# ml4ai/mliis

Measured on AMD Instinct MI355X. Metric: inner-loop images/sec (EfficientLab-6-3, 224x224, 5-shot), higher is better.
Workload: dtype f32 (the long-K decoder convs and their filter gradients with every operand split exactly into three bf16 terms on the matrix cores, 6 term products, f32 accumulate: fp32-equivalent products; everything else the fp32 instruction)

## Files before the change

### mliis_amd/csrc/bn.hip

```cpp
#include "common.hpp"
#include "se_wgrad.hpp"
#include "bn_fold.hpp"

namespace mliis {

constexpr int kColThreads = 256;
constexpr int kChanBlock = 32;
constexpr int kRowLanes = 32;
constexpr int kBatch = 4;
constexpr int kPoolRows = 128;
constexpr int kStatsPartialTarget = 256;

struct ColGeom {
  int gx;
  int rows_per_block;
  int nblk;
};

static inline ColGeom col_geom(long long rows_per_seg, int C, int nseg, int target_blocks = 2048) {
  ColGeom g;
  g.gx = ceil_div(C, kChanBlock);
  long long want = target_blocks / ((long long)g.gx * (nseg > 0 ? nseg : 1));
  if (want < 1) want = 1;
  long long rpb = (rows_per_seg + want - 1) / want;
  const long long unit = kRowLanes * kBatch;
  rpb = (rpb + unit - 1) / unit * unit;
  g.rows_per_block = (int)rpb;
  g.nblk = ceil_div(rows_per_seg, rpb);
  return g;
}

template <class Op>
__global__ __launch_bounds__(kColThreads) void colreduce_partial_k(Op op, int rows_per_seg, int C, int rows_per_block, int nblk,
                                                                    float* __restrict__ part) {
  constexpr int NV = Op::NV;
  __shared__ float4 sm[NV][4][8];
  const int t = threadIdx.x;
  const int q = t & 7, rl = t >> 3;
  const int c = blockIdx.y * kChanBlock + q * 4;
  const int seg = blockIdx.z;
  const bool active = c < C;
  float4 acc[NV];
#pragma unroll
  for (int v = 0; v < NV; ++v) acc[v] = f4zero();
  if (active) {
    const int r0 = blockIdx.x * rows_per_block;
    int r1 = r0 + rows_per_block;
    if (r1 > rows_per_seg) r1 = rows_per_seg;
    const long long base = (long long)seg * rows_per_seg;
    int r = r0 + rl;
    typename Op::Raw first[kBatch];
#pragma unroll
    for (int u = 0; u < kBatch; ++u) {
      const int ru = r + u * kRowLanes;
      op.load(seg, base + (ru < r1 ? ru : r0), c, first[u]);
    }
    const typename Op::Ctx ctx = op.ctx(c);
#pragma unroll
    for (int u = 0; u < kBatch; ++u)
      if (r + u * kRowLanes < r1) {
        float4 vals[NV];
        op.eval(ctx, first[u], vals);
#pragma unroll
        for (int v = 0; v < NV; ++v) acc[v] = f4add(acc[v], vals[v]);
// ... 2 lines not shown
    for (; r + (kBatch - 1) * kRowLanes < r1; r += kBatch * kRowLanes) {
      typename Op::Raw raw[kBatch];
#pragma unroll
      for (int u = 0; u < kBatch; ++u) op.load(seg, base + r + u * kRowLanes, c, raw[u]);
#pragma unroll
      for (int u = 0; u < kBatch; ++u) {
        float4 vals[NV];
        op.eval(ctx, raw[u], vals);
#pragma unroll
        for (int v = 0; v < NV; ++v) acc[v] = f4add(acc[v], vals[v]);
      }
    }
    for (; r < r1; r += kRowLanes) {
      typename Op::Raw raw;
      op.load(seg, base + r, c, raw);
      float4 vals[NV];
      op.eval(ctx, raw, vals);
#pragma unroll
      for (int v = 0; v < NV; ++v) acc[v] = f4add(acc[v], vals[v]);
    }
  }
#pragma unroll
  for (int v = 0; v < NV; ++v) {
#pragma unroll
    for (int off = 8; off < 64; off <<= 1) {
      acc[v].x += __shfl_xor(acc[v].x, off);
      acc[v].y += __shfl_xor(acc[v].y, off);
      acc[v].z += __shfl_xor(acc[v].z, off);
      acc[v].w += __shfl_xor(acc[v].w, off);
    }
    if ((t & 63) < 8) sm[v][t >> 6][q] = acc[v];
  }
  __syncthreads();
  if (t < 8 * NV) {
    const int v = t >> 3, qq = t & 7;
    const int cc = blockIdx.y * kChanBlock + qq * 4;
    if (cc < C) {
      float4 s4 = f4add(f4add(sm[v][0][qq], sm[v][1][qq]), f4add(sm[v][2][qq], sm[v][3][qq]));
      st4(part + (((long long)seg * nblk + blockIdx.x) * NV + v) * C + cc, s4);
    }
  }
}

template <class Op>
static int launch_colreduce(Op op, long long rows_per_seg, int C, int nseg, float* part, size_t part_floats,
                            hipStream_t stream, ColGeom* out_g, const char* name, int target_blocks = 2048) {
  ColGeom g = col_geom(rows_per_seg, C, nseg, target_blocks);
  size_t need = (size_t)nseg * g.nblk * Op::NV * C;
  MLIIS_REQUIRE(need <= part_floats, MLIIS_ERR_WORKSPACE, "%s: workspace too small (%zu floats needed, %zu given)", name,
                need, part_floats);
  dim3 grid(g.nblk, g.gx, nseg);
  hipLaunchKernelGGL((colreduce_partial_k<Op>), grid, dim3(kColThreads), 0, stream, op, (int)rows_per_seg, C, g.rows_per_block, g.nblk,
                     part);
  MLIIS_CHECK_LAUNCH(name);
  *out_g = g;
  return MLIIS_OK;
}

struct StatsOp {
  static constexpr int NV = 2;
  const float* x;
  int ld;
  int pre_swish;
  typedef float4 Raw;
  struct Ctx {};
  __device__ __forceinline__ Ctx ctx(int) const { return Ctx(); }
  __device__ __forceinline__ void load(int, long long row, int c, Raw& r) const { r = ld4(x + row * ld + c); }
// ... 437 lines not shown
  }
  __device__ __forceinline__ void eval(const Ctx& k, const Raw& r, float4* o) const {
    float a[5], b[5], c[5], d[5];
    one(r.x.x, r.g.x, k.m.x, k.rs.x, k.ga.x, k.be.x, a);
    one(r.x.y, r.g.y, k.m.y, k.rs.y, k.ga.y, k.be.y, b);
    one(r.x.z, r.g.z, k.m.z, k.rs.z, k.ga.z, k.be.z, c);
    one(r.x.w, r.g.w, k.m.w, k.rs.w, k.ga.w, k.be.w, d);
#pragma unroll
    for (int v = 0; v < 5; ++v) o[v] = make_float4(a[v], b[v], c[v], d[v]);
  }
};

struct Outer2Op {
  static constexpr int NV = 2;
  const float* x;
  int ldx;
  const float* mask;
  const float* dy;
  struct Raw { float4 x, m; float2 d; };
  struct Ctx {};
  __device__ __forceinline__ Ctx ctx(int) const { return Ctx(); }
  __device__ __forceinline__ void load(int, long long row, int c, Raw& r) const {
    r.x = ld4(x + row * ldx + c);
    r.m = mask != nullptr ? ld4(mask + row * ldx + c) : make_float4(1.f, 1.f, 1.f, 1.f);
    r.d = *reinterpret_cast<const float2*>(dy + row * 2);
  }
  __device__ __forceinline__ void eval(const Ctx&, const Raw& r, float4* o) const {
    const float4 v = f4mul(r.x, r.m);
    o[0] = f4scale(v, lone(r.d.x));
    o[1] = f4scale(v, lone(r.d.y));
  }
};

__global__ __launch_bounds__(256) void sum_finalize_k(const float* __restrict__ part, int nblk, int NV, int C, int nseg, float scale,
                                                      float* __restrict__ out, int accumulate) {
  __shared__ double sm[kFoldY * (kFoldX + 1)];
  const int c = blockIdx.x * kFoldX + threadIdx.x;
  const int v = blockIdx.y, seg = blockIdx.z;
  const bool ok = c < C;
  const double s = fold_partials(part + (long long)seg * nblk * NV * C, nblk, (long long)NV * C, (long long)v * C + c, ok, sm);
  if (!ok || threadIdx.y != 0) return;
  const long long i = ((long long)seg * NV + v) * C + c;
  const float r = (float)(s * (double)scale);
  out[i] = accumulate ? out[i] + r : r;
}

constexpr int kFoldTile = 256;

__global__ __launch_bounds__(256) void fold_batched_k(const float* __restrict__ part_base, float* __restrict__ out_base,
                                                      const long long* __restrict__ desc, int ndesc, long long fold_tiles,
                                                      const long long* __restrict__ se_desc, int n_se) {
  __shared__ double sm[3][64][4];
  const long long tile = blockIdx.x;
  if (tile >= fold_tiles) {
    se_wgrad_tile(se_desc, n_se, tile - fold_tiles);
    return;
  }
  int lo = 0, hi = ndesc - 1;
  while (lo < hi) {
    const int mid = (lo + hi + 1) >> 1;
    if (desc[(long long)mid * 8 + 7] <= tile) lo = mid; else hi = mid - 1;
  }
  const long long* d = desc + (long long)lo * 8;
  const long long total = d[2];
  const int nblk = (int)d[6];
  const int t = threadIdx.x, ql = t & 63, sl = t >> 6;
  const long long i = (tile - d[7]) * kFoldTile + ql * 4;
  const bool vec = ((total | d[0]) & 3) == 0;
  const float* p = part_base + d[0] + i;
  double a0 = 0, a1 = 0, a2 = 0, a3 = 0;
  if (i < total) {
    if (vec) {
      int k = sl;
      for (; k + 60 < nblk; k += 64) {
        float4 v[16];
#pragma unroll
        for (int u = 0; u < 16; ++u) v[u] = ld4(p + (long long)(k + 4 * u) * total);
#pragma unroll
        for (int u = 0; u < 16; ++u) { a0 += v[u].x; a1 += v[u].y; a2 += v[u].z; a3 += v[u].w; }
      }
      for (; k + 12 < nblk; k += 16) {
        float4 v[4];
#pragma unroll
        for (int u = 0; u < 4; ++u) v[u] = ld4(p + (long long)(k + 4 * u) * total);
#pragma unroll
        for (int u = 0; u < 4; ++u) { a0 += v[u].x; a1 += v[u].y; a2 += v[u].z; a3 += v[u].w; }
      }
      for (; k < nblk; k += 4) {
        const float4 v = ld4(p + (long long)k * total);
        a0 += v.x; a1 += v.y; a2 += v.z; a3 += v.w;
      }
    } else {
      for (int k = sl; k < nblk; k += 4) {
        const float* pk = p + (long long)k * total;
        a0 += pk[0];
        if (i + 1 < total) a1 += pk[1];
        if (i + 2 < total) a2 += pk[2];
        if (i + 3 < total) a3 += pk[3];
      }
// ... 458 lines not shown
        a1 += (double)d[u].y + (double)d[u].w;
      }
    }
    if ((rows & 1) && t == 0) {
      a0 += dy[(rows - 1) * 2];
      a1 += dy[(rows - 1) * 2 + 1];
    }
    sb[0][t] = a0;
    sb[1][t] = a1;
    __syncthreads();
    for (int s_ = 128; s_ > 0; s_ >>= 1) {
      if (t < s_) {
        sb[0][t] += sb[0][t + s_];
        sb[1][t] += sb[1][t + s_];
      }
      __syncthreads();
    }
    if (t == 0) {
      db[0] = (float)sb[0][0];
      db[1] = (float)sb[1][0];
    }
    return;
  }
  const int c = blockIdx.x * kFoldX + threadIdx.x;
  const int j = blockIdx.y;
  const bool ok = c < C;
  const double s = fold_partials(part, nblk, 2LL * C, (long long)j * C + c, ok, sm);
  if (ok && threadIdx.y == 0) dw[c * 2 + j] = (float)s;
}
}

extern "C" int mliis_final_conv_bwd_filter(const float* x, int ldx, const float* mask, const float* dy, long long rows, int C,
                                           float* dw, float* db, float* ws, size_t ws_floats, hipStream_t stream) {
  MLIIS_REQUIRE(x && dy && dw && db && ws, MLIIS_ERR_ARG, "final_conv_bwd_filter: null pointer");
  MLIIS_REQUIRE(rows > 0 && C > 0 && (C & 3) == 0 && (ldx & 3) == 0 && ldx >= C, MLIIS_ERR_ARG, "final_conv_bwd_filter: bad shape");
  MLIIS_REQUIRE(aligned16(x) && aligned16(mask) && aligned16(ws) && aligned16(dy), MLIIS_ERR_ALIGN, "final_conv_bwd_filter: alignment");
  Outer2Op op{x, ldx, mask, dy};
  ColGeom g;
  int rc = launch_colreduce(op, rows, C, 1, ws, ws_floats, stream, &g, "final_conv_bwd_filter");
  if (rc) return rc;
  hipLaunchKernelGGL(final_dw_finalize_k, dim3(ceil_div(C, kFoldX), 3), dim3(kFoldX, kFoldY), 0, stream, ws, g.nblk, C, dw, dy, rows, db);
  MLIIS_CHECK_LAUNCH("final_dw_finalize");
  return MLIIS_OK;
}
```

### mliis_amd/csrc/se.hip

```cpp
#include "common.hpp"
#include "se_wgrad.hpp"

namespace mliis {

constexpr int kMaxR = 128;
constexpr int kSeThreads = 1024;

template <int U>
__device__ __forceinline__ float dot_strided(const float* __restrict__ a, int sa, const float* __restrict__ b, long long sb, int n) {
  float acc = 0.f;
  for (int i = 0; i < n; i += U) {
    float x[U], y[U];
#pragma unroll
    for (int u = 0; u < U; ++u) {
      const int k = i + u < n ? i + u : n - 1;
      x[u] = a[(long long)k * sa];
      y[u] = b[(long long)k * sb];
    }
#pragma unroll
    for (int u = 0; u < U; ++u) acc = fmaf(i + u < n ? x[u] : 0.f, y[u], acc);
  }
  return acc;
}

// ... 303 lines not shown
    const long long r = ru;
    const long long n = ru / (unsigned)rows_per_img;
    float* dst = y + r * ldy + c;
    const float4 vx = ld4(x ? x + r * ldx + c : dst);
    const float4 vs = ld4(S ? S + n * C + c : dst);
    const float4 va = ld4(A ? A + n * C + c : dst);
    const float4 vo = ld4(dst);
    float4 v = x ? vx : f4zero();
    if (S) v = f4mul(v, vs);
    if (A) v = f4add(v, va);
    if (accumulate) v = f4add(v, vo);
    st4(dst, v);
  }
}

__global__ __launch_bounds__(256) void chan_split_k(const float* __restrict__ x, int ldx, const float* __restrict__ A, float* __restrict__ y0,
                                                    int ld0, int c0, int acc0, float* __restrict__ y1, int ld1, int acc1, long long rows, int C,
                                                    int rows_per_img) {
  const unsigned Q = (unsigned)C >> 2;
  const unsigned total = (unsigned)rows * Q;
  for (unsigned i = blockIdx.x * blockDim.x + threadIdx.x; i < total; i += gridDim.x * blockDim.x) {
    const unsigned ru = i / Q;
    const int c = (int)(i - ru * Q) << 2;
    const long long r = ru;
    const long long n = ru / (unsigned)rows_per_img;
    const bool first = c < c0;
    float* dst = first ? y0 + r * ld0 + c : y1 + r * ld1 + (c - c0);
    const bool acc = first ? acc0 != 0 : acc1 != 0;
    const float4 vx = ld4(x + r * ldx + c);
    const float4 va = ld4(A ? A + n * C + c : x + r * ldx + c);
    const float4 vo = ld4(dst);
    float4 v = vx;
    if (A) v = f4add(v, va);
    if (acc) v = f4add(v, vo);
    st4(dst, v);
  }
}

}

using namespace mliis;

extern "C" {

int mliis_se_mlp_fwd(const float* s_part, int chunks, float scale, float* s_out, const float* w1, const float* b1, const float* w2,
                     const float* b2, float* hpre, float* gate, int N, int C, int R, hipStream_t stream) {
  MLIIS_REQUIRE(s_part && w1 && b1 && w2 && b2 && hpre && gate, MLIIS_ERR_ARG, "se_mlp_fwd: null pointer");
  MLIIS_REQUIRE(N > 0 && C > 0 && C <= 8192 && R > 0 && R <= kMaxR && chunks > 0, MLIIS_ERR_ARG, "se_mlp_fwd: bad shape (R <= %d, C <= 8192)",
                kMaxR);
  const int CL = kSeThreads / R;
  if (C <= kSeThreads && R <= 32 && (C + CL - 1) / CL <= kSeFastDot)
    hipLaunchKernelGGL(se_mlp_fwd_k<true>, dim3(N), dim3(kSeThreads), (size_t)C * sizeof(float), stream, s_part, chunks, scale, s_out, w1, b1, w2,
                       b2, hpre, gate, C, R);
  else
    hipLaunchKernelGGL(se_mlp_fwd_k<false>, dim3(N), dim3(kSeThreads), (size_t)C * sizeof(float), stream, s_part, chunks, scale, s_out, w1, b1, w2,
                       b2, hpre, gate, C, R);
  MLIIS_CHECK_LAUNCH("se_mlp_fwd");
  return MLIIS_OK;
}

int mliis_se_mlp_bwd(const float* dgate, int dgate_row_groups, const float* gate, const float* s, const float* hpre, const float* w1,
                     const float* w1t, const float* w2, float* dpre1, float* dpre2, float* chan_add, float* dw1, float* db1, float* dw2, float* db2, int N,
                     int C, int R, int HW, hipStream_t stream) {
  MLIIS_REQUIRE(dgate_row_groups == 0 || (HW >= 16 && (long long)dgate_row_groups * 16 >= (long long)N * HW), MLIIS_ERR_ARG,
                "se_mlp_bwd: the row-group partials do not cover the N * HW rows (maps of at least 16 pixels)");
  MLIIS_REQUIRE(dgate && gate && s && hpre && w1 && w2 && dpre1 && dpre2 && chan_add, MLIIS_ERR_ARG, "se_mlp_bwd: null pointer (w1t alone may be NULL)");
// ... 16 lines not shown
}

int mliis_se_mlp_bwd_bn(const float* sums, int sums_nblk, const float* gate, const float* hpre, const float* w1, const float* w1t, const float* w2,
                        float* dpre1, float* dpre2, float* chan_add, float* stage1, int N, int C, int R, int HW, hipStream_t stream) {
  MLIIS_REQUIRE(sums && sums_nblk > 0 && gate && hpre && w1 && w2 && dpre1 && dpre2 && chan_add && stage1, MLIIS_ERR_ARG, "se_mlp_bwd_bn: null pointer");
  MLIIS_REQUIRE(N > 0 && C > 0 && C <= 8192 && R > 0 && R <= kMaxR && HW > 0, MLIIS_ERR_ARG, "se_mlp_bwd_bn: bad shape (R <= %d, C <= 8192)", kMaxR);
  if (C <= kSeThreads && R <= 32)
    hipLaunchKernelGGL(se_mlp_bwd_k<true>, dim3(N), dim3(kSeThreads), (size_t)(5 * C + 5 * kSeThreads) * sizeof(float), stream, nullptr, 0, HW, gate, hpre, w1,
                       w1t, w2, dpre2,
                       dpre1, chan_add, C, R, 1.0f / (float)HW, sums, sums_nblk, stage1);
  else
    hipLaunchKernelGGL(se_mlp_bwd_k<false>, dim3(N), dim3(kSeThreads), (size_t)5 * C * sizeof(float), stream, nullptr, 0, HW, gate, hpre, w1, w1t, w2, dpre2,
                       dpre1, chan_add, C, R, 1.0f / (float)HW, sums, sums_nblk, stage1);
  MLIIS_CHECK_LAUNCH("se_mlp_bwd_bn");
  return MLIIS_OK;
}

int mliis_se_wgrad_batched(const long long* desc, int ndesc, long long total_tiles, hipStream_t stream) {
  MLIIS_REQUIRE(desc && ndesc > 0 && total_tiles > 0, MLIIS_ERR_ARG, "se_wgrad_batched: bad arguments");
  hipLaunchKernelGGL(se_wgrad_batched_k, dim3((unsigned)total_tiles), dim3(256), 0, stream, desc, ndesc);
  MLIIS_CHECK_LAUNCH("se_wgrad_batched");
  return MLIIS_OK;
}

int mliis_chan_split(const float* x, int ldx, const float* A, float* y0, int ld0, int c0, int accumulate0, float* y1, int ld1, int accumulate1,
                     long long rows, int C, int rows_per_img, hipStream_t stream) {
  MLIIS_REQUIRE(x && y0 && y1, MLIIS_ERR_ARG, "chan_split: null pointer");
  MLIIS_REQUIRE(rows > 0 && C > 0 && (C & 3) == 0 && c0 > 0 && c0 < C && (c0 & 3) == 0 && (ldx & 3) == 0 && ldx >= C && (ld0 & 3) == 0 &&
                    ld0 >= c0 && (ld1 & 3) == 0 && ld1 >= C - c0 && rows_per_img > 0,
                MLIIS_ERR_ARG, "chan_split: bad shape");
  MLIIS_REQUIRE(aligned16(x) && aligned16(A) && aligned16(y0) && aligned16(y1), MLIIS_ERR_ALIGN, "chan_split: pointers must be 16-byte aligned");
  MLIIS_REQUIRE(rows * (C / 4) < (1LL << 31), MLIIS_ERR_UNSUPPORTED, "chan_split: tensor too large for 32-bit indexing");
  long long q = rows * (C / 4);
  int blocks = (int)((q + 255) / 256 > 4096 ? 4096 : (q + 255) / 256);
  hipLaunchKernelGGL(chan_split_k, dim3(blocks), dim3(256), 0, stream, x, ldx, A, y0, ld0, c0, accumulate0, y1, ld1, accumulate1, rows, C,
                     rows_per_img);
  MLIIS_CHECK_LAUNCH("chan_split");
  return MLIIS_OK;
}

int mliis_chan_affine(const float* x, int ldx, const float* S, const float* A, float* y, int ldy, long long rows, int C,
                      int rows_per_img, int accumulate, hipStream_t stream) {
  MLIIS_REQUIRE(y && (x || A), MLIIS_ERR_ARG, "chan_affine: need an output and at least one of x / A");
  MLIIS_REQUIRE(rows > 0 && C > 0 && (C & 3) == 0 && (ldy & 3) == 0 && ldy >= C && rows_per_img > 0 &&
                    (x == nullptr || ((ldx & 3) == 0 && ldx >= C)),
                MLIIS_ERR_ARG, "chan_affine: bad shape");
  MLIIS_REQUIRE(aligned16(x) && aligned16(S) && aligned16(A) && aligned16(y), MLIIS_ERR_ALIGN, "chan_affine: pointers must be 16-byte aligned");
  MLIIS_REQUIRE(rows * (C / 4) < (1LL << 31), MLIIS_ERR_UNSUPPORTED, "chan_affine: tensor too large for 32-bit indexing");
  long long q = rows * (C / 4);
  int blocks = (int)((q + 255) / 256 > 4096 ? 4096 : (q + 255) / 256);
  hipLaunchKernelGGL(chan_affine_k, dim3(blocks), dim3(256), 0, stream, x, ldx, S, A, y, ldy, rows, C, rows_per_img, accumulate);
  MLIIS_CHECK_LAUNCH("chan_affine");
  return MLIIS_OK;
}
}
```

### mliis_amd/ops.py

```python
from __future__ import annotations

import ctypes as C
import os
from typing import Optional, Tuple

import torch

from ._lib import MliisError, lib
from .spec import BN_EPS, BN_MOMENTUM, MEAN_RGB, STDDEV_RGB

_MEAN3 = (C.c_float * 3)(*MEAN_RGB)
_STD3 = (C.c_float * 3)(*STDDEV_RGB)


def _stream() -> int:
    return torch.cuda.current_stream().cuda_stream


def _ptr(t: Optional[torch.Tensor]):
    if t is None:
        return None
    if not t.is_cuda:
        raise MliisError("mliis_amd ops need device tensors (no CPU path)")
    if t.dtype == torch.bfloat16:
# ... 1001 lines not shown
    lib.call("mliis_resize_bilinear_bwd", _ptr(dy), lddy, _ptr(out), lddx, N, Hi, Wi, Ho, Wo, C_, int(accumulate), _stream())
    return out


def final_conv_fwd(x, w, b, mask=None, out=None):
    rows, C_, ldx = rows_ld(x)
    _dense(w, b, mask)
    if mask is not None and mask.numel() != rows * C_:
        raise MliisError("final_conv_fwd: mask must be a dense [rows, {}] tensor, got {}".format(C_, tuple(mask.shape)))
    _out_dense(out, tuple(x.shape[:-1]) + (2,), what="final_conv_fwd out")
    out = torch.empty(tuple(x.shape[:-1]) + (2,), dtype=torch.float32, device=x.device) if out is None else out
    lib.call("mliis_final_conv_fwd", _ptr(x), ldx, _ptr(mask), _ptr(w), _ptr(b), _ptr(out), rows, C_, _stream())
    return out


def final_conv_bwd_data(dy, w, C_, mask=None, out=None, fin=None):
    rows = dy.numel() // 2
    _dense(dy, w, mask)
    if mask is not None and mask.numel() != rows * C_:
        raise MliisError("final_conv_bwd_data: mask must be a dense [rows, {}] tensor, got {}".format(C_, tuple(mask.shape)))
    _out_rows(out, tuple(dy.shape[:-1]) + (C_,), what="final_conv_bwd_data out")
    out = torch.empty(tuple(dy.shape[:-1]) + (C_,), dtype=torch.float32, device=dy.device) if out is None else out
    _, _, lddx = rows_ld(out)
    if fin is not None:
        buf, size, extra_loss, loss_out = fin
        N, Hd, Wd = dy.shape[:3]
        lib.call("mliis_final_conv_bwd_data_fin", _ptr(dy), _ptr(w), _ptr(mask), _ptr(out), lddx, rows, C_, _ptr(buf), N, Hd, Wd, int(size[0]), int(size[1]),
                 float(extra_loss), _ptr(loss_out), _stream())
        return out
    lib.call("mliis_final_conv_bwd_data", _ptr(dy), _ptr(w), _ptr(mask), _ptr(out), lddx, rows, C_, _stream())
    return out


def final_conv_bwd_filter(x, dy, mask=None, dw=None, db=None, ws: Optional[Workspace] = None):
    rows, C_, ldx = rows_ld(x)
    _dense(dy, mask)
    if mask is not None and mask.numel() != rows * C_:
        raise MliisError("final_conv_bwd_filter: mask must be a dense [rows, {}] tensor, got {}".format(C_, tuple(mask.shape)))
    _out_dense(dw, (1, 1, C_, 2), what="final_conv_bwd_filter dw")
    _out_dense(db, (2,), what="final_conv_bwd_filter db")
    dw = torch.empty((1, 1, C_, 2), dtype=torch.float32, device=x.device) if dw is None else dw
    db = torch.empty(2, dtype=torch.float32, device=x.device) if db is None else db
    ws = ws or default_ws()
    buf = ws.get(lib.size("mliis_colreduce_workspace_floats", rows, C_, 1, 2))
    lib.call("mliis_final_conv_bwd_filter", _ptr(x), ldx, _ptr(mask), _ptr(dy), rows, C_, _ptr(dw), _ptr(db), _ptr(buf), buf.numel(), _stream())
    return dw, db


def softmax_ce(logits, labels, idx=None, label_smoothing=0.0, dice=False, extra_loss=0.0, want_grad=True, want_pred=False, dlogits=None,
               pred=None, out=None, ws: Optional[Workspace] = None):
    N, H, W, _ = logits.shape
    dev = logits.device
    _dense(logits, labels, idx)
    _out_dense(dlogits, tuple(logits.shape), what="softmax_ce dlogits")
    _out_dense(pred, tuple(logits.shape), what="softmax_ce pred")
    if want_grad and dlogits is None:
        dlogits = torch.empty_like(logits)
    if want_pred and pred is None:
        pred = torch.empty_like(logits)
    out = torch.empty(4, dtype=torch.float32, device=dev) if out is None else out
    ws = ws or default_ws()
    buf = ws.get(lib.size("mliis_softmax_ce_workspace_floats", N, H, W))
    lib.call("mliis_softmax_ce", _ptr(logits), _ptr(labels), _ptr(idx), N, H, W, float(label_smoothing), int(dice), float(extra_loss),
             _ptr(dlogits) if want_grad else None, _ptr(pred) if want_pred else None, _ptr(out), _ptr(buf), buf.numel(), _stream())
    return out, dlogits, pred


def head_ce_fused(small, labels, idx, size, label_smoothing, dsmall, out, extra_loss=0.0, ws: Optional[Workspace] = None, finalize=True):
    N, Hd, Wd, _ = small.shape
    _dense(small, labels, idx)
    _out_dense(dsmall, tuple(small.shape), what="head_ce_fused dsmall")
# ... 82 lines not shown
```

### mliis_amd/passes.py

```python
from __future__ import annotations

import torch

from . import ops, spec
from ._lib import MliisError
from .plan import _Plan


class _Pass:

    def __init__(self, L, P: _Plan, training: bool):
        self.L, self.P, self.training = L, P, training
        self.w, self.mv, self.g, self.ws = L.arena.w, L.arena.mv, L.arena.g, L.ws

    def moving(self, prefix):
        return self.mv[prefix + "/moving_mean"], self.mv[prefix + "/moving_variance"]

    def bn_bwd_args(self, st, prefix):
        return st[0], st[1], self.w[prefix + "/gamma"], self.w[prefix + "/beta"]

    def bn_fwd_args(self, st, prefix, moving=True):
        return (self.w[prefix + "/gamma"], self.w[prefix + "/beta"], st[0], st[1]) + (self.moving(prefix) if moving else (None, None))

    def moving_stats(self, st, prefix):
# ... 264 lines not shown
        a, A, ws, T, N = self.arch, self.arena, self.ws, P.aspp, P.N
        w, g = A.w, A.g
        d, hw = a.aspp_dimension, a.aspp_h * a.aspp_h
        (k0, c0), (k1, c1), (k2, c2), (ko, co) = self.n_aspp
        m = T["masks"]
        cat, dcat = T["cat"], T["dcat"]
        dzo = ops.swish_mask_bwd(T["dout"], T["zo"], m[3], out=T["dzo"])
        self._conv_bwd_filter(cat, dzo, 1, 1, out=g[ko], ws=ws)
        ops.colsum(dzo, out=g[co], ws=ws)
        self._conv_bwd_data(dzo, w[ko], 1, out=dcat, ws=ws)
        d0 = ops.swish_mask_bwd(dcat[..., 2 * d:], T["z0"], m[0], out=dcat[..., 2 * d:])
        self._conv_bwd_filter(x, d0, 1, 1, out=g[k0], ws=ws)
        ops.colsum(d0, out=g[c0], ws=ws)
        self._conv_bwd_data(d0, w[k0], 1, out=dx, accumulate=dx_has, ws=ws)
        d1 = ops.swish_mask_bwd(dcat[..., d:2 * d], T["z1"], m[1], out=dcat[..., d:2 * d])
        self._conv_bwd_filter(x, d1, 3, spec.ASPP_DILATION, out=g[k1], ws=ws)
        ops.colsum(d1, out=g[c1], ws=ws)
        self._conv_bwd_data(d1, w[k1], spec.ASPP_DILATION, out=dx, accumulate=True, ws=ws)
        ops.colsum(dcat[..., :d], None, nseg=N, out=T["db2"], ws=ws)
        d2 = ops.swish_mask_bwd(T["db2"], T["z2"], m[2], out=T["db2"], pre_mask=True)
        pool4, d24 = T["pool"].view(N, 1, 1, -1), d2.view(N, 1, 1, d)
        self._conv_bwd_filter(pool4, d24, 1, 1, out=g[k2], ws=ws)
        ops.colsum(d2, out=g[c2], ws=ws)
        self._conv_bwd_data(d24, w[k2], 1, out=T["dpool"].view(N, 1, 1, -1), ws=ws)
        ops.axpby(0.0, None, 1.0 / hw, T["dpool"])
        ops.chan_affine(None, A=T["dpool"], out=dx, accumulate=True)

    def _backward(self, P: _Plan, x, idx, head_fused: bool = False):
        a, S = self.arch, _Pass(self, P, True)
        w, g = S.w, S.g
        if not head_fused:
            ops.resize_bilinear_bwd(P.dlogits, (a.h_dec, a.h_dec), out=P.dsmall)
        mask = P.drop_mask
        ops.final_conv_bwd_filter(P.dec_in, P.dsmall, mask, dw=g[self.n_final[0]], db=g[self.n_final[1]], ws=S.ws)
        has_grad = [False] * len(P.blocks)
        dtop, _ = self._deep_grad_target(P, has_grad, len(a.rsd))
        ops.final_conv_bwd_data(P.dsmall, w[self.n_final[0]], a.c_final, mask, out=dtop, fin=P.head_fin if head_fused else None)
        if not P.wbatch_ready:
            P.wbatch = ops.FilterBatch(self.device)
        for j in range(len(a.rsd) - 1, -1, -1):
            self._rsd_bwd(S, j, has_grad)
        if a.skipdec is not None:
            self._skipdec_bwd(S, has_grad)
        if a.aspp:
            bi = a.reductions[4]
            self._aspp_backward(P, P.blocks[bi]["out"], P.blocks[bi]["dout"], has_grad[bi])
            has_grad[bi] = True
        stage1 = None
        ex = a.executed()
        for bi in range(len(P.blocks) - 1, -1, -1):
            b, B, nm = ex[bi], P.blocks[bi], self.n_blocks[bi]
            if not has_grad[bi]:
                raise MliisError("internal: block {} has no upstream gradient".format(bi))
            tgt = P.blocks[bi - 1]["dout"] if bi > 0 else P.dstem
            tgt_has = has_grad[bi - 1] if bi > 0 else False
            if B["small"]:
                stage1 = self._mbconv_small_bwd(S, bi, b, B, nm, tgt, tgt_has, stage1)
            elif B["march"]:
                stage1 = self._mbconv_march_bwd(S, bi, b, B, nm, tgt, tgt_has, stage1)
            else:
                stage1 = self._mbconv_opbyop_bwd(S, bi, b, B, nm, tgt, tgt_has, stage1)
            if bi > 0:
                has_grad[bi - 1] = True
        self._stem_bwd(S, x, idx, stage1)
        P.wbatch_ready = True
        P.wbatch.launch("fp32x3" if self.x3 is not None else self.matmul_precision)
        ops.fold_batched(P.fold_buf, self.arena.grad, P.fold_desc, P.fold_tiles, se_desc=P.se_desc, se_tiles=P.se_tiles)

    def _deep_grad_target(self, P: _Plan, has_grad, j):
        a = self.arch
        if j > 0:
            return P.rsd[j - 1]["dout"], False
        if j == 0 and a.skipdec is not None:
            return P.skipdec["dout"], False
        if a.aspp:
            return P.aspp["dout"], False
        bi = a.reductions[4]
        tgt_has, has_grad[bi] = has_grad[bi], True
        return P.blocks[bi]["dout"], tgt_has

    def _rsd_bwd(self, S: _Pass, j, has_grad):
        a, P, w, g, ws = self.arch, S.P, S.w, S.g, S.ws
        m, D, nm = a.rsd[j], P.rsd[j], self.n_rsd[j]
        (k0, b0, n0), (k1, b1, n1), (kf, bf, nf) = nm
        co = m.c_out
        dO, cat, pyr, dpyr, dcat = D["dout"], D["cat"], D["pyr"], D["dpyr"], D["dcat"]
        S.bn_b(D["zf"], dO, D["stf"], nf, D["dzf"], pre=True)
        ops.rsd_pool_bwd(D["dzf"], D["tot"], D["pool"], w[kf], 2 * co, dw=g[kf], dbias=g[bf], dpool=D["dpool"], ws=ws)
        S.wgrad_conv(pyr, D["dzf"], 3, 1, kf)
        S.conv_bwd_data(D["dzf"], kf, 1, 2 * co, dpyr)
        d0, d1 = dpyr[..., :co], dpyr[..., co:2 * co]
        ops.bn_bwd_pair([(D["z" + i], d_, *S.bn_bwd_args(D["st" + i], nn), d_, g[nn + "/gamma"], g[nn + "/beta"], P.fold_part[bb])
                         for i, d_, nn, bb in (("0", d0, n0, b0), ("1", d1, n1, b1))], pre_swish=True, ws=ws)
        tail = P.filter_tail[j]
        cmain = cat[..., :m.c_cat - tail] if tail else cat

        def wgrad(dz, kname, kk, dil, cmain=cmain, ctail=cat[..., m.c_cat - tail:] if tail else None):
            S.wgrad_conv(cmain, dz, kk, dil, kname)
            if ctail is not None:
                S.wgrad_conv(ctail, dz, kk, dil, kname + "#tail")
        wgrad(d0, k0, 1, 1)
        self._conv_bwd_data(d0, w[k0], 1, out=dcat, ws=ws)
        wgrad(d1, k1, 3, 2)
        S.conv_bwd_data(d1, k1, 2, m.c_cat, dcat, accumulate=True)
        bi_skip = a.reductions[m.scope_index + 1]
        if m.upsample_conv:
            ku, bu, nu = self.n_rsd_up[j]
            S.bn_b(D["zu"], dO, D["stu"], nu, D["dzu"], pre=True, dxsum_part=P.fold_part[bu])
            S.wgrad_conv(cat[..., :m.c_deep], D["dzu"], 1, 1, ku)
            self._conv_bwd_data(D["dzu"], w[ku], 1, out=D["dup"], ws=ws)
            dU = D["dup"]
        else:
            dU = dO
        ops.chan_split(dcat, m.c_deep, dU, True, P.blocks[bi_skip]["dout"], has_grad[bi_skip], A=D["dpool"])
        has_grad[bi_skip] = True
        tgt, tgt_has = self._deep_grad_target(P, has_grad, j)
        if m.h_in == m.h:
            ops.chan_affine(dU, out=tgt, accumulate=tgt_has)
        else:
            ops.resize_bilinear_bwd(dU, (m.h_in, m.h_in), out=tgt, accumulate=tgt_has)

    def _skipdec_bwd(self, S: _Pass, has_grad):
        a, P, w, ws = self.arch, S.P, S.w, S.ws
        sd, T = a.skipdec, P.skipdec
        (k0, n0), seps = self.n_skipdec
        d = T["dout"]
        for Q, (dwn, dbn, pwn, pbn) in zip(reversed(T["sep"]), reversed(seps)):
            S.bn_b(Q["zp"], d, Q["stp"], pbn, d, post=True)
            S.wgrad_conv(Q["ad"], d, 1, 1, pwn)
            self._conv_bwd_data(d, w[pwn], 1, out=Q["dad"], ws=ws)
            S.bn_b(Q["zd"], Q["dad"], Q["std"], dbn, Q["dad"], post=True)
            ops.dwconv_bwd_filter(Q["x_in"], Q["dad"], 3, 1, partial=P.fold_part[dwn])
            ops.dwconv_bwd_data(Q["dad"], w[dwn], 1, (sd.h, sd.h), out=Q["din"])
            d = Q["din"]
        bi2 = a.reductions[2]
        S.bn_b(T["z0"], d[..., sd.c_in:], T["st0"], n0, T["dz0"], post=True)
        S.wgrad_conv(P.blocks[bi2]["out"], T["dz0"], 1, 1, k0)
        self._conv_bwd_data(T["dz0"], w[k0], 1, out=P.blocks[bi2]["dout"], accumulate=has_grad[bi2], ws=ws)
# ... 96 lines not shown
```

### mliis_amd/plan.py

```python
from __future__ import annotations

import torch

from . import ops, spec
from ._lib import MliisError, lib


class _Plan:

    def __init__(self, L: "Learner", N: int, act_dtype=torch.float32):
        a, dev = L.arch, L.device
        self.N = N
        self.act_dtype = act_dtype

        def buf(*shape):
            return torch.empty(shape, dtype=torch.float32, device=dev)

        def xbuf(*shape):
            return torch.empty(shape, dtype=act_dtype, device=dev)

        def vec(c):
            return buf(c), buf(c)
        self.idx = torch.zeros(N, dtype=torch.int32, device=dev)
        H = a.image_size
# ... 89 lines not shown
        if a.skipdec is not None:
            rows = N * a.skipdec.h ** 2
            for c in (a.skipdec.c_skip, a.skipdec.c_cat, a.skipdec.c_sep):
                need = max(need, -(-rows // 16) * 2 * c, ops.bn_stats_partial_floats(rows, c))
        need = max(need, ops.bn_stats_partial_floats(N * hs * hs, a.stem_out), ops.stem_conv_fwd_stats_floats(N, H, H, a.stem_out))
        self.stats_part = buf(need + 64)
        need2 = 0
        for b in a.executed():
            need2 = max(need2, lib.raw("mliis_dwconv_bn_fwd_blocks")(N, b.h_in, b.h_in, b.cexp, b.k, b.stride) * 2 * b.cexp,
                        lib.raw("mliis_dwconv_bn_bwd_blocks")(N, b.h_in, b.h_in, b.cexp, b.k, b.stride) * 2 * b.cexp)
        for m in a.rsd:
            need2 = max(need2, -(-(N * m.h * m.h) // 16) * 2 * m.c_out, ops.bn_stats_partial_floats(N * m.h * m.h, m.c_out))
        self.stats_part2 = buf(need2 + 64)
        ex_ = a.executed()
        self.bn2_deferred = [bool(L.fuse_bn2 and i + 1 < len(ex_) and ex_[i + 1].expand != 1 and act_dtype in (torch.float32, torch.bfloat16) and
                                  ops.conv2d_fwd_bnin_ok(N, ex_[i].h_out, ex_[i].h_out, ex_[i].cout, ex_[i + 1].cexp)) for i in range(len(ex_))]
        self.stats_part3 = buf(max([-(-(N * b.h_out ** 2) // 16) * 2 * b.cout for b, d in zip(ex_, self.bn2_deferred) if d] + [0]) + 64)
        self.sums_part = buf(max([ops.se_bn_bwd_sums_floats(N, b.h_out * b.h_out, b.cexp) for b in a.executed()] + [0]) + 64)
        self.stage1_se = buf(max([2 * N * b.cexp for b in a.executed()] + [0]) + 64)
        self.pool_part = buf(max(N * (-(-(b.h_out * b.h_out) // 128)) * b.cexp for b in a.executed()) + 64)
        self.gate_part = buf(max([(-(-(N * b.h_out * b.h_out) // 16)) * 2 * b.cexp for b in a.executed() if 16 <= b.h_out * b.h_out <= 256]
                                 + [0]) + 64)
        A = L.arena
        regs, rows, off, tile = {}, [], 0, 0
        fold_tile = lib.raw("mliis_fold_tile_outputs")()

        def add(name, ws_floats, total, seg=None, key=None):
            nonlocal off, tile
            seg_len, seg_stride, seg_off = seg or (total, 0, 0)
            regs[key or name] = (off, ws_floats)
            rows.append([off, A.t_off[name], total, seg_len, seg_stride, seg_off, ws_floats // total, tile])
            off += (ws_floats + 3) // 4 * 4
            tile += -(-total // fold_tile)
        fe = a.name
        add(f"{fe}/stem/conv2d/kernel", lib.size("mliis_stem_conv_bwd_filter_workspace_floats", N, H, H, a.stem_out), 27 * a.stem_out)
        for b, nm, B in zip(a.executed(), L.n_blocks, self.blocks):
            ce = b.cexp
            if b.expand != 1:
                add(nm["w_exp"], lib.size("mliis_conv2d_bwd_filter_workspace_floats", N, b.h_in, b.h_in, b.cin, ce, 1), b.cin * ce)
            if B["march"]:
                add(nm["w_dw"], lib.raw("mliis_dwconv_bn_bwd_blocks")(N, b.h_in, b.h_in, ce, b.k, b.stride) * b.k * b.k * ce, b.k * b.k * ce)
            elif not B["small"]:
                add(nm["w_dw"], lib.size("mliis_dwconv_bwd_filter_workspace_floats", N, b.h_in, b.h_in, ce, b.k, b.stride), b.k * b.k * ce)
            add(nm["w_proj"], lib.size("mliis_conv2d_bwd_filter_workspace_floats", N, b.h_out, b.h_out, ce, b.cout, 1), ce * b.cout)
        if a.skipdec is not None:
            sd, h = a.skipdec, a.skipdec.h
            ksk, seps = L.n_skipdec
            add(ksk[0], lib.size("mliis_conv2d_bwd_filter_workspace_floats", N, h, h, sd.c_skip_in, sd.c_skip, 1), sd.c_skip_in * sd.c_skip)
            cin = sd.c_cat
            for (dwn, _, pwn, _) in seps:
                add(dwn, lib.size("mliis_dwconv_bwd_filter_workspace_floats", N, h, h, cin, 3, 1), 9 * cin)
                add(pwn, lib.size("mliis_conv2d_bwd_filter_workspace_floats", N, h, h, cin, sd.c_sep, 1), cin * sd.c_sep)
                cin = sd.c_sep
        self.filter_tail = {}
        for j_rsd, (m, nm) in enumerate(zip(a.rsd, L.n_rsd)):
            (k0, b0_, _), (k1, b1_, _), (kf, _, _) = nm
            co = m.c_out
            if m.upsample_conv:
                ku, bu, _ = L.n_rsd_up[j_rsd]
                add(ku, lib.size("mliis_conv2d_bwd_filter_workspace_floats", N, m.h, m.h, m.c_deep, co, 1), m.c_deep * co)
                add(bu, ops.bn_bwd_dxsum_floats(N * m.h * m.h, co), co)
            for bias in (b0_, b1_):
                add(bias, ops.bn_bwd_dxsum_floats(N * m.h * m.h, co), co)
            tail = m.c_cat % 64 if (m.c_cat > 64 and 0 < m.c_cat % 64 <= 16) else 0
            self.filter_tail[j_rsd] = tail
            for kk, kname in ((1, k0), (3, k1)):
                main_c = m.c_cat - tail
                add(kname, lib.size("mliis_conv2d_bwd_filter_workspace_floats", N, m.h, m.h, main_c, co, kk), kk * kk * main_c * co,
                    seg=(main_c * co, m.c_cat * co, 0) if tail else None)
                if tail:
                    add(kname, lib.size("mliis_conv2d_bwd_filter_workspace_floats", N, m.h, m.h, tail, co, kk), kk * kk * tail * co,
                        seg=(tail * co, m.c_cat * co, main_c * co), key=kname + "#tail")
            add(kf, lib.size("mliis_conv2d_bwd_filter_workspace_floats", N, m.h, m.h, 2 * co, co, 3), 9 * 2 * co * co,
                seg=(2 * co * co, m.c_pyr * co, 0))
        rows_se, se_tile = [], 0
        for b, B, nm in zip(a.executed(), self.blocks, L.n_blocks):
            se = nm["se"]
            rows_se.append([B["s"].data_ptr(), B["hpre"].data_ptr(), B["dpre1"].data_ptr(), B["dpre2"].data_ptr()] +
                           [A.g[k].data_ptr() for k in se] + [N, b.cexp, b.se, se_tile])
            se_tile += -(-(2 * b.cexp * b.se + b.cexp + b.se) // 256)
        self.se_desc = torch.tensor(rows_se, dtype=torch.int64, device=dev)
        self.se_tiles = se_tile
        self.fold_buf = buf(off + 16)
        self.fold_part = {k: self.fold_buf[o:o + n] for k, (o, n) in regs.items()}
        self.fold_desc = torch.tensor(rows, dtype=torch.int64, device=dev)
        self.fold_tiles = tile
        self.graphs = {}
        self.steps_run = 0
        self.wbatch = ops.FilterBatch(dev)
        self.wbatch_ready = False
        jobs = []
        if L.drop_connect and nskip:
            jobs.append((self.dc_all, L._dc_keeps, N, True))
        if self.drop_mask is not None:
            jobs.append((self.drop_mask, L.drop_keep_dev, self.drop_mask.numel(), False))
        if self.aspp is not None:
            for mbuf in self.aspp["masks"]:
                jobs.append((mbuf, 1.0 - spec.ASPP_DROPOUT, 1, False))
        self.mask_plan = ops.MaskPlan(jobs) if jobs else None

    @property
    def graph(self):
        for g in self.graphs.values():
            return g
        return None
```

Baseline: 3586.

## Fold final conv filter partials in batched fold and fuse direct RSD skip grads

The final 1x1 conv filter gradient now writes its per-block partial slabs, including the bias sums as an extra vector, straight into the shared fold buffer. A new tiny-total path in fold_batched_k reduces them there, which removes the separate finalize launch. The RSD backward, when there is no upsampling and the resolutions match, now routes the skip gradient through bn_b's dskip output. It also adds a chan_split variant that writes both channel halves into one target, summing them in a single pass. Together these cut kernel launches and intermediate buffer traffic, at the cost of more special-case code paths.

After: 3596, median of 6. About the same (+0.3%).

```diff
diff --git a/mliis_amd/csrc/bn.hip b/mliis_amd/csrc/bn.hip
--- a/mliis_amd/csrc/bn.hip
+++ b/mliis_amd/csrc/bn.hip
@@ -30,6 +30,11 @@
   return g;
 }
 
+template <class Op, class = void>
+struct StoresFinalSlabs { static constexpr bool value = false; };
+template <class Op>
+struct StoresFinalSlabs<Op, decltype((void)Op::kFinalSlabs)> { static constexpr bool value = true; };
+
 template <class Op>
 __global__ __launch_bounds__(kColThreads) void colreduce_partial_k(Op op, int rows_per_seg, int C, int rows_per_block, int nblk,
                                                                     float* __restrict__ part) {
@@ -98,7 +103,23 @@
     if ((t & 63) < 8) sm[v][t >> 6][q] = acc[v];
   }
   __syncthreads();
-  if (t < 8 * NV) {
+  if constexpr (StoresFinalSlabs<Op>::value) {
+    if (t < 8) {
+      const int cc = blockIdx.y * kChanBlock + t * 4;
+      if (cc < C) {
+        const float4 s0 = f4add(f4add(sm[0][0][t], sm[0][1][t]), f4add(sm[0][2][t], sm[0][3][t]));
+        const float4 s1 = f4add(f4add(sm[1][0][t], sm[1][1][t]), f4add(sm[1][2][t], sm[1][3][t]));
+        float* o = part + ((long long)blockIdx.x * C + cc) * 2;
+        st4(o, make_float4(s0.x, s1.x, s0.y, s1.y));
+        st4(o + 4, make_float4(s0.z, s1.z, s0.w, s1.w));
+      }
+    } else if (t == 8 && blockIdx.y == 0) {
+      const float4 s2 = f4add(f4add(sm[2][0][0], sm[2][1][0]), f4add(sm[2][2][0], sm[2][3][0]));
+      float* o = part + (long long)nblk * 2 * C + (long long)blockIdx.x * 2;
+      o[0] = s2.x;
+      o[1] = s2.y;
+    }
+  } else if (t < 8 * NV) {
     const int v = t >> 3, qq = t & 7;
     const int cc = blockIdx.y * kChanBlock + qq * 4;
     if (cc < C) {
@@ -602,6 +623,15 @@
   }
 };
 
+struct Outer2SlabOp : Outer2Op {
+  static constexpr int NV = 3;
+  static constexpr bool kFinalSlabs = true;
+  __device__ __forceinline__ void eval(const Ctx& k, const Raw& r, float4* o) const {
+    Outer2Op::eval(k, r, o);
+    o[2] = make_float4(r.d.x, r.d.y, 0.f, 0.f);
+  }
+};
+
 __global__ __launch_bounds__(256) void sum_finalize_k(const float* __restrict__ part, int nblk, int NV, int C, int nseg, float scale,
                                                       float* __restrict__ out, int accumulate) {
   __shared__ double sm[kFoldY * (kFoldX + 1)];
@@ -635,6 +665,27 @@
   const long long total = d[2];
   const int nblk = (int)d[6];
   const int t = threadIdx.x, ql = t & 63, sl = t >> 6;
+  if (total <= 4) {
+    double a[4] = {0.0, 0.0, 0.0, 0.0};
+    for (int k = t; k < nblk; k += 256) {
+      const float* pk = part_base + d[0] + (long long)k * total;
+#pragma unroll
+      for (int e = 0; e < 4; ++e)
+        if (e < total) a[e] += pk[e];
+    }
+#pragma unroll
+    for (int e = 0; e < 4; ++e) {
+#pragma unroll
+      for (int off = 1; off < 64; off <<= 1) a[e] += __shfl_xor(a[e], off);
+      if (ql == 0) sm[0][sl][e] = a[e];
+    }
+    __syncthreads();
+    if (t < total) {
+      const long long seg_len = d[3];
+      out_base[d[1] + (t / seg_len) * d[4] + d[5] + t % seg_len] = (float)((sm[0][0][t] + sm[0][1][t]) + (sm[0][2][t] + sm[0][3][t]));
+    }
+    return;
+  }
   const long long i = (tile - d[7]) * kFoldTile + ql * 4;
   const bool vec = ((total | d[0]) & 3) == 0;
   const float* p = part_base + d[0] + i;
@@ -1159,9 +1210,20 @@
 
 extern "C" int mliis_final_conv_bwd_filter(const float* x, int ldx, const float* mask, const float* dy, long long rows, int C,
                                            float* dw, float* db, float* ws, size_t ws_floats, hipStream_t stream) {
-  MLIIS_REQUIRE(x && dy && dw && db && ws, MLIIS_ERR_ARG, "final_conv_bwd_filter: null pointer");
+  MLIIS_REQUIRE(x && dy && ws && (dw == nullptr) == (db == nullptr), MLIIS_ERR_ARG, "final_conv_bwd_filter: null pointer (dw and db come together)");
   MLIIS_REQUIRE(rows > 0 && C > 0 && (C & 3) == 0 && (ldx & 3) == 0 && ldx >= C, MLIIS_ERR_ARG, "final_conv_bwd_filter: bad shape");
   MLIIS_REQUIRE(aligned16(x) && aligned16(mask) && aligned16(ws) && aligned16(dy), MLIIS_ERR_ALIGN, "final_conv_bwd_filter: alignment");
+  if (dw == nullptr) {
+    const ColGeom gs = col_geom(rows, C, 1);
+    const size_t need = (size_t)gs.nblk * (2 * (size_t)C + 2);
+    MLIIS_REQUIRE(need <= ws_floats, MLIIS_ERR_WORKSPACE, "final_conv_bwd_filter: slab buffer too small (%zu floats needed, %zu given)", need, ws_floats);
+    Outer2SlabOp sop;
+    sop.x = x; sop.ldx = ldx; sop.mask = mask; sop.dy = dy;
+    hipLaunchKernelGGL((colreduce_partial_k<Outer2SlabOp>), dim3(gs.nblk, gs.gx, 1), dim3(kColThreads), 0, stream, sop, (int)rows, C, gs.rows_per_block,
+                       gs.nblk, ws);
+    MLIIS_CHECK_LAUNCH("final_conv_bwd_filter (slabs)");
+    return MLIIS_OK;
+  }
   Outer2Op op{x, ldx, mask, dy};
   ColGeom g;
   int rc = launch_colreduce(op, rows, C, 1, ws, ws_floats, stream, &g, "final_conv_bwd_filter");
diff --git a/mliis_amd/csrc/se.hip b/mliis_amd/csrc/se.hip
--- a/mliis_amd/csrc/se.hip
+++ b/mliis_amd/csrc/se.hip
@@ -359,6 +359,33 @@
     const float4 vo = ld4(dst);
     float4 v = vx;
     if (A) v = f4add(v, va);
+    if (acc) v = f4add(v, vo);
+    st4(dst, v);
+  }
+}
+
+__global__ __launch_bounds__(256) void chan_split_same_k(const float* __restrict__ x, int ldx, const float* __restrict__ A, float* __restrict__ y,
+                                                         int ldy, int c0, int acc, long long rows, int C, int rows_per_img) {
+  const int c1 = C - c0;
+  const unsigned Q = (unsigned)(c0 > c1 ? c0 : c1) >> 2;
+  const unsigned total = (unsigned)rows * Q;
+  for (unsigned i = blockIdx.x * blockDim.x + threadIdx.x; i < total; i += gridDim.x * blockDim.x) {
+    const unsigned ru = i / Q;
+    const int c = (int)(i - ru * Q) << 2;
+    const long long r = ru;
+    const long long n = ru / (unsigned)rows_per_img;
+    const bool h0 = c < c0, h1 = c < c1;
+    const int ca = h0 ? c : c0 + c, cb = h1 ? c0 + c : c;
+    float* dst = y + r * ldy + c;
+    const float4 xa = ld4(x + r * ldx + ca), xb = ld4(x + r * ldx + cb);
+    const float4 aa = ld4(A ? A + n * C + ca : x + r * ldx + ca), ab = ld4(A ? A + n * C + cb : x + r * ldx + cb);
+    const float4 vo = ld4(dst);
+    float4 va = xa, vb = xb;
+    if (A) {
+      va = f4add(va, aa);
+      vb = f4add(vb, ab);
+    }
+    float4 v = h0 ? (h1 ? f4add(va, vb) : va) : vb;
     if (acc) v = f4add(v, vo);
     st4(dst, v);
   }
@@ -441,6 +468,15 @@
   MLIIS_REQUIRE(aligned16(x) && aligned16(A) && aligned16(y0) && aligned16(y1), MLIIS_ERR_ALIGN, "chan_split: pointers must be 16-byte aligned");
   MLIIS_REQUIRE(rows * (C / 4) < (1LL << 31), MLIIS_ERR_UNSUPPORTED, "chan_split: tensor too large for 32-bit indexing");
   long long q = rows * (C / 4);
+  if (y0 == y1) {
+    MLIIS_REQUIRE(ld0 == ld1 && (accumulate0 != 0) == (accumulate1 != 0), MLIIS_ERR_ARG,
+                  "chan_split: y0 == y1 needs one leading dimension and one accumulate setting");
+    q = rows * ((c0 > C - c0 ? c0 : C - c0) / 4);
+    hipLaunchKernelGGL(chan_split_same_k, dim3((int)((q + 255) / 256 > 4096 ? 4096 : (q + 255) / 256)), dim3(256), 0, stream, x, ldx, A, y0, ld0, c0,
+                       accumulate0, rows, C, rows_per_img);
+    MLIIS_CHECK_LAUNCH("chan_split (one target)");
+    return MLIIS_OK;
+  }
   int blocks = (int)((q + 255) / 256 > 4096 ? 4096 : (q + 255) / 256);
   hipLaunchKernelGGL(chan_split_k, dim3(blocks), dim3(256), 0, stream, x, ldx, A, y0, ld0, c0, accumulate0, y1, ld1, accumulate1, rows, C,
                      rows_per_img);
diff --git a/mliis_amd/ops.py b/mliis_amd/ops.py
--- a/mliis_amd/ops.py
+++ b/mliis_amd/ops.py
@@ -1057,11 +1057,21 @@
     return out
 
 
-def final_conv_bwd_filter(x, dy, mask=None, dw=None, db=None, ws: Optional[Workspace] = None):
+def final_conv_bwd_filter_slabs(rows, C_):
+    nb = lib.size("mliis_colreduce_workspace_floats", rows, C_, 1, 2) // (2 * C_)
+    return nb, nb * (2 * C_ + 2)
+
+
+def final_conv_bwd_filter(x, dy, mask=None, dw=None, db=None, ws: Optional[Workspace] = None, slabs=None):
     rows, C_, ldx = rows_ld(x)
-    _dense(dy, mask)
+    _dense(dy, mask, slabs)
     if mask is not None and mask.numel() != rows * C_:
         raise MliisError("final_conv_bwd_filter: mask must be a dense [rows, {}] tensor, got {}".format(C_, tuple(mask.shape)))
+    if slabs is not None:
+        if dw is not None or db is not None:
+            raise MliisError("final_conv_bwd_filter: slabs are folded by fold_batched -- dw / db are not written by this form")
+        lib.call("mliis_final_conv_bwd_filter", _ptr(x), ldx, _ptr(mask), _ptr(dy), rows, C_, None, None, _ptr(slabs), slabs.numel(), _stream())
+        return final_conv_bwd_filter_slabs(rows, C_)[0]
     _out_dense(dw, (1, 1, C_, 2), what="final_conv_bwd_filter dw")
     _out_dense(db, (2,), what="final_conv_bwd_filter db")
     dw = torch.empty((1, 1, C_, 2), dtype=torch.float32, device=x.device) if dw is None else dw
diff --git a/mliis_amd/passes.py b/mliis_amd/passes.py
--- a/mliis_amd/passes.py
+++ b/mliis_amd/passes.py
@@ -320,7 +320,7 @@
         if not head_fused:
             ops.resize_bilinear_bwd(P.dlogits, (a.h_dec, a.h_dec), out=P.dsmall)
         mask = P.drop_mask
-        ops.final_conv_bwd_filter(P.dec_in, P.dsmall, mask, dw=g[self.n_final[0]], db=g[self.n_final[1]], ws=S.ws)
+        ops.final_conv_bwd_filter(P.dec_in, P.dsmall, mask, slabs=P.final_slabs)
         has_grad = [False] * len(P.blocks)
         dtop, _ = self._deep_grad_target(P, has_grad, len(a.rsd))
         ops.final_conv_bwd_data(P.dsmall, w[self.n_final[0]], a.c_final, mask, out=dtop, fin=P.head_fin if head_fused else None)
@@ -373,7 +373,10 @@
         (k0, b0, n0), (k1, b1, n1), (kf, bf, nf) = nm
         co = m.c_out
         dO, cat, pyr, dpyr, dcat = D["dout"], D["cat"], D["pyr"], D["dpyr"], D["dcat"]
-        S.bn_b(D["zf"], dO, D["stf"], nf, D["dzf"], pre=True)
+        direct = m.h_in == m.h and not m.upsample_conv
+        if direct:
+            tgt, tgt_has = self._deep_grad_target(P, has_grad, j)
+        S.bn_b(D["zf"], dO, D["stf"], nf, D["dzf"], pre=True, dskip=tgt if direct else None, dskip_accumulate=direct and tgt_has)
         ops.rsd_pool_bwd(D["dzf"], D["tot"], D["pool"], w[kf], 2 * co, dw=g[kf], dbias=g[bf], dpool=D["dpool"], ws=ws)
         S.wgrad_conv(pyr, D["dzf"], 3, 1, kf)
         S.conv_bwd_data(D["dzf"], kf, 1, 2 * co, dpyr)
@@ -392,6 +395,10 @@
         wgrad(d1, k1, 3, 2)
         S.conv_bwd_data(d1, k1, 2, m.c_cat, dcat, accumulate=True)
         bi_skip = a.reductions[m.scope_index + 1]
+        if direct:
+            ops.chan_split(dcat, m.c_deep, tgt, True, P.blocks[bi_skip]["dout"], has_grad[bi_skip], A=D["dpool"])
+            has_grad[bi_skip] = True
+            return
         if m.upsample_conv:
             ku, bu, nu = self.n_rsd_up[j]
             S.bn_b(D["zu"], dO, D["stu"], nu, D["dzu"], pre=True, dxsum_part=P.fold_part[bu])
diff --git a/mliis_amd/plan.py b/mliis_amd/plan.py
--- a/mliis_amd/plan.py
+++ b/mliis_amd/plan.py
@@ -145,6 +145,9 @@
             rows.append([off, A.t_off[name], total, seg_len, seg_stride, seg_off, ws_floats // total, tile])
             off += (ws_floats + 3) // 4 * 4
             tile += -(-total // fold_tile)
+        nb_f, _ = ops.final_conv_bwd_filter_slabs(N * hd * hd, a.c_final)
+        add(L.n_final[0], nb_f * 2 * a.c_final, 2 * a.c_final)
+        add(L.n_final[1], nb_f * 2, 2)
         fe = a.name
         add(f"{fe}/stem/conv2d/kernel", lib.size("mliis_stem_conv_bwd_filter_workspace_floats", N, H, H, a.stem_out), 27 * a.stem_out)
         for b, nm, B in zip(a.executed(), L.n_blocks, self.blocks):
@@ -196,6 +199,7 @@
         self.se_tiles = se_tile
         self.fold_buf = buf(off + 16)
         self.fold_part = {k: self.fold_buf[o:o + n] for k, (o, n) in regs.items()}
+        self.final_slabs = self.fold_buf[regs[L.n_final[0]][0]:regs[L.n_final[1]][0] + nb_f * 2]
         self.fold_desc = torch.tensor(rows, dtype=torch.int64, device=dev)
         self.fold_tiles = tile
         self.graphs = {}
```
